# okieraised/rs-face-detection-tflite

Measured on AMD Instinct MI355X. Metric: faces/sec at batch=256 (256x256 back-camera) per GPU, higher is better.
Workload: dtype f32

## Files before the change

### rs-face-detection-tflite_amd/csrc/chain_kernels.hip

```cpp
#include <hip/hip_runtime.h>

#include <algorithm>
#include <cstdint>
#include <type_traits>

#include "kernels.hpp"
#include "launch.hpp"

namespace mi {

typedef float f32x16c __attribute__((ext_vector_type(16)));
typedef float f32x2c __attribute__((ext_vector_type(2)));

namespace {

__device__ __forceinline__ float4 cld4(const float* p) { return *reinterpret_cast<const float4*>(p); }

struct ChainGeom {
    int Cp, Ch, C4, PS, RS, MT;
    int off_wdw, off_bdw, off_bias, off_alpha;
    int split;
    int pre_P, pre_RP, pre_GP, pre_PS, pre_RS;
    int off_t8;
    int lds_bytes;
    unsigned long long* stamps;
};
#ifdef MI_CHAIN_STAMPS
unsigned long long* g_chain_stamps = nullptr;
#define MI_CHAIN_STAMP(k) if (g.stamps && threadIdx.x == 0) { __builtin_amdgcn_sched_barrier(0); g.stamps[(long)blockIdx.x * 24 + (k)] = __builtin_amdgcn_s_memtime(); __builtin_amdgcn_sched_barrier(0); }
#else
#define MI_CHAIN_STAMP(k)
#endif

constexpr int chain_pre_passes(int C, int H, int W, int Cin, int post_Co, int MT, bool split, long tile) {
    const int pre_RS = (2 * W + 1) * (Cin + 4);
    for (int P = 1; P <= 4; P++) {
        const int RP = (H + P - 1) / P, GP = (RP * W + 31) / 32;
        const long stage = (long)(2 * RP + 1) * pre_RS;
        const long rest = 9 * C + C + 8 * 32 + 64 + (post_Co ? (long)(H >> 1) * (W >> 1) * (post_Co + 4) : 0);
        if ((P - 1) * RP < H && P * GP * (split ? MT : 1) <= 8 && ((stage > tile ? stage : tile) + rest) * 4 <= 160 * 1024 - 256) return P;
    }
    return 0;
}

struct GeomRun {
// ... 21 lines not shown
    static constexpr bool all_res = true;
    struct K {
        static constexpr int C = C_, H = H_, W = W_, Cp = C, Ch = C / 2, C4 = C / 4, PS = C + 4, RS = (W + 2) * PS, MT = (C + 31) / 32;
        static constexpr bool split = MT > 1 && ((H * W + 31) / 32) * MT <= 8;
        static constexpr int pre_on = CIN != 0, pre_Cin = CIN, post_on = CO != 0, post_Co = CO;
        static constexpr int tile = (H + 2) * RS;
        static constexpr int pre_PS = CIN + 4, pre_RS = (2 * W + 1) * pre_PS;
        static constexpr int pre_P = CIN ? chain_pre_passes(C, H, W, CIN, CO, MT, split, tile) : 0;
        static constexpr int pre_RP = CIN ? (H + pre_P - 1) / pre_P : 0, pre_GP = (pre_RP * W + 31) / 32;
        static constexpr int stage = CIN ? (2 * pre_RP + 1) * pre_RS : 0;
        static constexpr int off_wdw = stage > tile ? stage : tile, off_bdw = off_wdw + 9 * Cp, off_bias = (off_bdw + Cp + 3) & ~3;
        static constexpr int off_alpha = off_bias + MT * 32;
    };
    static_assert(!CIN || K::pre_P > 0, "no staging plan for `pre`");
    __device__ GeomFixed(const ChainArgs&, const ChainGeom&) {}
#define MI_GEOM_FIELD(f) static constexpr __device__ int f() { return K::f; }
    MI_GEOM_FIELD(C) MI_GEOM_FIELD(H) MI_GEOM_FIELD(W) MI_GEOM_FIELD(pre_on) MI_GEOM_FIELD(pre_Cin) MI_GEOM_FIELD(post_on) MI_GEOM_FIELD(post_Co)
    MI_GEOM_FIELD(Cp) MI_GEOM_FIELD(Ch) MI_GEOM_FIELD(C4) MI_GEOM_FIELD(PS) MI_GEOM_FIELD(RS)
    MI_GEOM_FIELD(off_wdw) MI_GEOM_FIELD(off_bdw) MI_GEOM_FIELD(off_bias) MI_GEOM_FIELD(off_alpha)
    MI_GEOM_FIELD(pre_P) MI_GEOM_FIELD(pre_RP) MI_GEOM_FIELD(pre_GP) MI_GEOM_FIELD(pre_PS) MI_GEOM_FIELD(pre_RS)
#undef MI_GEOM_FIELD
    static bool matches(const ChainArgs& a, const ChainGeom& g) {
        bool ok = a.C == K::C && a.H == K::H && a.W == K::W && g.Cp == K::Cp && g.Ch == K::Ch && g.C4 == K::C4 && g.PS == K::PS && g.RS == K::RS &&
                  g.MT == K::MT && (g.split != 0) == K::split && g.off_wdw == K::off_wdw && g.off_bdw == K::off_bdw && g.off_bias == K::off_bias &&
                  g.off_alpha == K::off_alpha && (a.pre.on != 0) == (CIN != 0) && (a.post.on != 0) == (CO != 0);
        if (ok && CIN) ok = a.pre.Cin == CIN && g.pre_P == K::pre_P && g.pre_RP == K::pre_RP && g.pre_GP == K::pre_GP && g.pre_PS == K::pre_PS && g.pre_RS == K::pre_RS;
        if (ok && CO) ok = a.post.Co == CO;
        for (int k = 0; ok && k < a.nblocks; k++) ok = a.blocks[k].has_res != 0;
        return ok;
    }
};
constexpr int kActRun = -1;

template <int MT, bool SPLIT, class GP = GeomRun, int ACT = kActRun>
__global__ __launch_bounds__(512, 2) void chain_kernel(ChainArgs a, ChainGeom g) {
    extern __shared__ __attribute__((aligned(16))) float lds[];
    const GP geo(a, g);
    float* tile = lds;
    const int tid = threadIdx.x, lane = tid & 63, wave = tid >> 6;
    const int pl = lane & 31, h = lane >> 5;
    const int b = blockIdx.x;
    const float* in = a.in + (long)b * a.in_fs;
    const int rowf4 = geo.W() * geo.C4();
    const int nch = geo.Ch() >> 2;

    struct ConstRegs { float w[3], bdw, bias, alpha; };
    auto fetch_consts = [&](const ChainBlock& cb, int Cs, int Cos, ConstRegs& r) {
#pragma unroll
        for (int k = 0; k < 3; k++) {
            const int i = tid + 512 * k, c = i % geo.Cp();
            r.w[k] = (i < 9 * geo.Cp() && c < Cs) ? cb.w_dw[(i / geo.Cp()) * Cs + c] : 0.f;
        }
        r.bdw = (tid < Cs && cb.b_dw) ? cb.b_dw[tid] : 0.f;
        r.bias = (tid < Cos && cb.bias) ? cb.bias[tid] : 0.f;
        if constexpr (ACT == kActRun) r.alpha = (tid < Cos && cb.act == ACT_PRELU) ? cb.alpha[tid] : (cb.act == ACT_NONE ? 1.f : 0.f);
    };
    auto commit_consts = [&](const ConstRegs& r) {
#pragma unroll
        for (int k = 0; k < 3; k++)
            if (tid + 512 * k < 9 * geo.Cp()) lds[geo.off_wdw() + tid + 512 * k] = r.w[k];
        if (tid < geo.Cp()) lds[geo.off_bdw() + tid] = r.bdw;
        if (tid < MT * 32) {
            lds[geo.off_bias() + tid] = r.bias;
            if constexpr (ACT == kActRun) lds[geo.off_alpha() + tid] = r.alpha;
        }
    };
    unsigned aoff[MT];
// ... 63 lines not shown
        };
        if constexpr (kPeel) step(0, std::true_type{});
        for (int j = kPeel ? 1 : 0; j + 1 < nchk; j++) step(j, std::false_type{});
        mfma_chunk(av, bf, D, std::false_type{});
    };
    constexpr int NJ = MT * 4;
    auto contract1 = [&](const float* w_pw, int nchk, int mt, auto&& dw, f32x16c& D1) {
        const float* wa = w_pw + ((long)mt * nchk * 64 + lane) * 4;
        float4 aw[NJ];
#pragma unroll
        for (int j = 0; j < NJ; j++)
            if (j < nchk) aw[j] = cld4(wa + 256 * j);
        if constexpr (!GP::fixed) {
#pragma unroll
            for (int e = 0; e < 16; e++) D1[e] = 0.f;
        }
        float4 bf;
        dw(0, bf);
#pragma unroll
        for (int j = 0; j < NJ; j++)
            if (j < nchk) {
                float4 bn = bf;
                int jn = j + 1;
                asm volatile("" : "+s"(jn));
                if (j + 1 < nchk) dw(jn, bn);
                if (GP::fixed && j == 0) D1 = __builtin_amdgcn_mfma_f32_32x32x2f32(aw[j].x, bf.x, zero16, 0, 0, 0);
                else D1 = __builtin_amdgcn_mfma_f32_32x32x2f32(aw[j].x, bf.x, D1, 0, 0, 0);
                D1 = __builtin_amdgcn_mfma_f32_32x32x2f32(aw[j].y, bf.y, D1, 0, 0, 0);
                D1 = __builtin_amdgcn_mfma_f32_32x32x2f32(aw[j].z, bf.z, D1, 0, 0, 0);
                D1 = __builtin_amdgcn_mfma_f32_32x32x2f32(aw[j].w, bf.w, D1, 0, 0, 0);
                bf = bn;
                __builtin_amdgcn_sched_barrier(0);
            }
    };
    auto finish1 = [&](f32x16c& D1, int ch, int gq, const float4& skip, float hi) {
        if constexpr (ACT == ACT_RELU) {
            const f32x2c* bb = reinterpret_cast<const f32x2c*>(lds + geo.off_bias() + ch);
            const f32x2c v0 = (f32x2c{D1[4 * gq], D1[4 * gq + 1]} + bb[0]) + f32x2c{skip.x, skip.y};
            const f32x2c v1 = (f32x2c{D1[4 * gq + 2], D1[4 * gq + 3]} + bb[1]) + f32x2c{skip.z, skip.w};
            D1[4 * gq] = fmaxf(v0.x, 0.f);
            D1[4 * gq + 1] = fmaxf(v0.y, 0.f);
            D1[4 * gq + 2] = fmaxf(v1.x, 0.f);
            D1[4 * gq + 3] = fmaxf(v1.y, 0.f);
            return;
        }
        const float4 bb = cld4(lds + geo.off_bias() + ch), al = cld4(lds + geo.off_alpha() + ch);
        const float4 v = make_float4(D1[4 * gq] + bb.x + skip.x, D1[4 * gq + 1] + bb.y + skip.y, D1[4 * gq + 2] + bb.z + skip.z, D1[4 * gq + 3] + bb.w + skip.w);
        D1[4 * gq] = fminf(fmaxf(v.x, 0.f) + al.x * fminf(v.x, 0.f), hi);
        D1[4 * gq + 1] = fminf(fmaxf(v.y, 0.f) + al.y * fminf(v.y, 0.f), hi);
        D1[4 * gq + 2] = fminf(fmaxf(v.z, 0.f) + al.z * fminf(v.z, 0.f), hi);
        D1[4 * gq + 3] = fminf(fmaxf(v.w, 0.f) + al.w * fminf(v.w, 0.f), hi);
    };
    const float4 zero4 = make_float4(0.f, 0.f, 0.f, 0.f);

    const int ngrp = (geo.H() * geo.W() + 31) >> 5;
    const int grp_w = SPLIT ? wave % ngrp : wave, mt_w = SPLIT ? wave / ngrp : 0;
    const int q = grp_w * 32 + pl;
    const bool valid = q < geo.H() * geo.W();
    const int oy = valid ? q / geo.W() : 0, ox = valid ? q - (q / geo.W()) * geo.W() : 0;
    const bool wave_active = SPLIT ? wave < ngrp * MT : wave * 32 < geo.H() * geo.W();
    const int base0 = oy * geo.RS() + ox * geo.PS() + h * geo.Ch();
    float* centre = tile + (oy + 1) * geo.RS() + (ox + 1) * geo.PS();

    MI_CHAIN_STAMP(0)
    ConstRegs cr;
    if (geo.pre_on()) {
// ... 17 lines not shown
            if (p) __syncthreads();
            for (int i = tid; i < nrows * rowf4i; i += 512) {
                const int rr = i / rowf4i, e = i - rr * rowf4i, px = e / C4i, c4 = e - px * C4i, iy = 2 * r0 + rr;
                *reinterpret_cast<float4*>(lds + rr * RSi + px * PSi + 4 * c4) = iy < Hi ? cld4(src + ((long)iy * rowf4i + e) * 4) : zero4;
            }
            for (int i = tid; i < nrows * C4i; i += 512) {
                const int rr = i / C4i, c4 = i - rr * C4i;
                *reinterpret_cast<float4*>(lds + rr * RSi + Wi * PSi + 4 * c4) = zero4;
            }
            __syncthreads();
            MI_CHAIN_STAMP(16 + p)
            const int u = wave - p * UP;
            if (u >= 0 && u < UP) {
                const int ugrp = SPLIT ? u % geo.pre_GP() : u, umt = SPLIT ? u / geo.pre_GP() : 0;
                const int qp = ugrp * 32 + pl;
                const bool vp = qp < (r1 - r0) * geo.W();
                const int oyl = vp ? qp / geo.W() : 0, oxp = vp ? qp - (qp / geo.W()) * geo.W() : 0;
                const float* t0 = lds + (2 * oyl) * RSi + (2 * oxp) * PSi;
                auto dw = [&](int j, float4& bf) {
                    const int c0 = h * Chp + 4 * j;
                    bf = cld4(bdw + c0);
#pragma unroll
                    for (int ky = 0; ky < 3; ky++)
#pragma unroll
                        for (int kx = 0; kx < 3; kx++) {
                            const float4 w = cld4(wdw + (ky * 3 + kx) * geo.Cp() + c0);
                            const float4 d = cld4(t0 + ky * RSi + kx * PSi + c0);
                            bf.x = fmaf(d.x, w.x, bf.x);
                            bf.y = fmaf(d.y, w.y, bf.y);
                            bf.z = fmaf(d.z, w.z, bf.z);
                            bf.w = fmaf(d.w, w.w, bf.w);
                        }
                };
                if constexpr (SPLIT) contract1(cb.w_pw, Chp >> 2, umt, dw, D[0]);
                else contract(cb, Chp >> 2, dw, D);
                const float hi = cb.act == ACT_RELU6 ? 6.f : INFINITY;
#pragma unroll
                for (int m = 0; m < (SPLIT ? 1 : MT); m++)
#pragma unroll
                    for (int gq = 0; gq < 4; gq++) {
                        const int ch = (SPLIT ? umt : m) * 32 + 8 * gq + 4 * h;
                        if (ch >= geo.C()) continue;
                        float4 sk = zero4;
                        if (cb.has_res && ch < Cin) {
                            const float4 s0 = cld4(t0 + ch), s1 = cld4(t0 + PSi + ch), s2 = cld4(t0 + RSi + ch), s3 = cld4(t0 + RSi + PSi + ch);
                            sk = make_float4(fmaxf(fmaxf(s0.x, s1.x), fmaxf(s2.x, s3.x)), fmaxf(fmaxf(s0.y, s1.y), fmaxf(s2.y, s3.y)),
                                             fmaxf(fmaxf(s0.z, s1.z), fmaxf(s2.z, s3.z)), fmaxf(fmaxf(s0.w, s1.w), fmaxf(s2.w, s3.w)));
                        }
                        finish1(D[m], ch, gq, sk, hi);
                    }
                mine = vp;
                my_mt = umt;
                my_centre = tile + (r0 + oyl + 1) * geo.RS() + (oxp + 1) * geo.PS();
            }
        }
        __syncthreads();
        for (int i = tid; i < ((geo.H() + 2) * geo.RS()) >> 2; i += 512) reinterpret_cast<float4*>(tile)[i] = zero4;
        commit_consts(cr);
        __syncthreads();
        if (mine) {
#pragma unroll
            for (int m = 0; m < (SPLIT ? 1 : MT); m++)
#pragma unroll
                for (int gq = 0; gq < 4; gq++) {
                    const int ch = (SPLIT ? my_mt : m) * 32 + 8 * gq + 4 * h;
                    if (ch < geo.C()) *reinterpret_cast<float4*>(my_centre + ch) = make_float4(D[m][4 * gq], D[m][4 * gq + 1], D[m][4 * gq + 2], D[m][4 * gq + 3]);
                }
// ... 35 lines not shown
                        for (int kx = 0; kx < 3; kx++) {
                            const float4 w = cld4(wj + (ky * 3 + kx) * geo.Cp());
                            const float4 d = cld4(tj + ky * geo.RS() + kx * geo.PS());
                            lo = __builtin_elementwise_fma(f32x2c{d.x, d.y}, f32x2c{w.x, w.y}, lo);
                            up = __builtin_elementwise_fma(f32x2c{d.z, d.w}, f32x2c{w.z, w.w}, up);
                        }
                    const float4 bb = cld4(wj + 9 * geo.Cp());
                    lo += f32x2c{bb.x, bb.y};
                    up += f32x2c{bb.z, bb.w};
                    bf = make_float4(lo.x, lo.y, up.x, up.y);
                    return;
                }
                const float* wj = wdw + h * geo.Ch() + 4 * j;
                bf = zero4;
#ifdef MI_ABL_CHAIN_NODW
                bf = cld4(tile + base0 + geo.RS() + geo.PS() + 4 * j);
                return;
#endif
#pragma unroll
                for (int ky = 0; ky < 3; ky++)
#pragma unroll
                    for (int kx = 0; kx < 3; kx++) {
                        const float4 w = cld4(wj + (ky * 3 + kx) * geo.Cp());
                        const float4 d = cld4(tile + base0 + ky * geo.RS() + kx * geo.PS() + 4 * j);
                        bf.x = fmaf(d.x, w.x, bf.x);
                        bf.y = fmaf(d.y, w.y, bf.y);
                        bf.z = fmaf(d.z, w.z, bf.z);
                        bf.w = fmaf(d.w, w.w, bf.w);
                    }
                const float4 bb = cld4(bdw + h * geo.Ch() + 4 * j);
                bf.x += bb.x; bf.y += bb.y; bf.z += bb.z; bf.w += bb.w;
            };
            const float hi = cb.act == ACT_RELU6 ? 6.f : INFINITY;
            if constexpr (SPLIT) contract1(cb.w_pw, nch, mt_w, dw, D[0]);
            else contract(cb, nch, dw, D);
#pragma unroll
            for (int m = 0; m < (SPLIT ? 1 : MT); m++)
#pragma unroll
                for (int gq = 0; gq < 4; gq++) {
                    const int ch = (SPLIT ? mt_w : m) * 32 + 8 * gq + 4 * h;
                    if (ch < geo.C()) finish1(D[m], ch, gq, (GP::all_res || cb.has_res) ? cld4(centre + ch) : zero4, hi);
                }
        }
        __syncthreads();
        if (more || geo.post_on()) commit_consts(cr);
        if (wave_active && valid) {
#pragma unroll
            for (int m = 0; m < (SPLIT ? 1 : MT); m++)
#pragma unroll
                for (int gq = 0; gq < 4; gq++) {
                    const int ch = (SPLIT ? mt_w : m) * 32 + 8 * gq + 4 * h;
                    if (ch < geo.C()) *reinterpret_cast<float4*>(centre + ch) = make_float4(D[m][4 * gq], D[m][4 * gq + 1], D[m][4 * gq + 2], D[m][4 * gq + 3]);
                }
        }
        __syncthreads();
        MI_CHAIN_STAMP(2 + blk)
    }
    if (a.write_out) {
        float* out = a.out + (long)b * a.out_fs;
        for (int i = tid; i < geo.H() * rowf4; i += 512) {
            int r = i / rowf4, e = i - r * rowf4;
            int px = e / geo.C4(), c4 = e - px * geo.C4();
            *reinterpret_cast<float4*>(out + 4 * (long)i) = cld4(tile + (r + 1) * geo.RS() + (px + 1) * geo.PS() + 4 * c4);
        }
    }
    MI_CHAIN_STAMP(10)
    int post_units = 0;
    if (geo.post_on()) {
        const ChainBlock& cb = a.post.blk;
        const int Ho = geo.H() >> 1, Wo = geo.W() >> 1, Co = geo.post_Co(), npo = Ho * Wo;
        const float* wdw = lds + geo.off_wdw();
        const float* bdw = lds + geo.off_bdw();
        const int ngo = (npo + 31) >> 5, MTo = (Co + 31) >> 5;
        post_units = ngo * MTo;
        for (int u = wave; u < post_units; u += 8) {
            const int grp = u % ngo, mt = u / ngo;
            const int qo = grp * 32 + pl;
            const bool vo = qo < npo;
            const int py = vo ? qo / Wo : 0, px = vo ? qo - (qo / Wo) * Wo : 0;
            const float* t0 = tile + (2 * py + 1) * geo.RS() + (2 * px + 1) * geo.PS();
            f32x16c D1;
            auto dw = [&](int j, float4& bf) {
                const int c0 = h * geo.Ch() + 4 * j;
                bf = cld4(bdw + c0);
#pragma unroll
                for (int ky = 0; ky < 3; ky++)
#pragma unroll
                    for (int kx = 0; kx < 3; kx++) {
                        const float4 w = cld4(wdw + (ky * 3 + kx) * geo.Cp() + c0);
                        const float4 d = cld4(t0 + ky * geo.RS() + kx * geo.PS() + c0);
                        bf.x = fmaf(d.x, w.x, bf.x);
                        bf.y = fmaf(d.y, w.y, bf.y);
                        bf.z = fmaf(d.z, w.z, bf.z);
                        bf.w = fmaf(d.w, w.w, bf.w);
                    }
            };
            contract1(cb.w_pw, nch, mt, dw, D1);
            const float hi = cb.act == ACT_RELU6 ? 6.f : INFINITY;
            float* dst = a.post.out + (long)b * a.post.out_fs + (long)qo * Co;
#pragma unroll
            for (int gq = 0; gq < 4; gq++) {
                const int ch = mt * 32 + 8 * gq + 4 * h;
                if (ch >= Co) continue;
                float4 sk = zero4;
                if (cb.has_res && ch < geo.C()) {
                    const float4 s0 = cld4(t0 + ch), s1 = cld4(t0 + geo.PS() + ch), s2 = cld4(t0 + geo.RS() + ch), s3 = cld4(t0 + geo.RS() + geo.PS() + ch);
                    sk = make_float4(fmaxf(fmaxf(s0.x, s1.x), fmaxf(s2.x, s3.x)), fmaxf(fmaxf(s0.y, s1.y), fmaxf(s2.y, s3.y)),
                                     fmaxf(fmaxf(s0.z, s1.z), fmaxf(s2.z, s3.z)), fmaxf(fmaxf(s0.w, s1.w), fmaxf(s2.w, s3.w)));
                }
                finish1(D1, ch, gq, sk, hi);
                if (vo) {
                    const float4 v = make_float4(D1[4 * gq], D1[4 * gq + 1], D1[4 * gq + 2], D1[4 * gq + 3]);
                    *reinterpret_cast<float4*>(dst + ch) = v;
                    if (g.off_t8 >= 0) *reinterpret_cast<float4*>(lds + g.off_t8 + qo * (Co + 4) + ch) = v;
                }
            }
        }
    }
    MI_CHAIN_STAMP(11)
    for (int hd = 0; hd < kChainHeads; hd++) {
        MI_CHAIN_STAMP(12 + hd)
        const ChainHead& H = a.heads[hd];
        if (!H.on) continue;
        if (H.src == 1) { __syncthreads(); post_units = 0; }
        const bool from_post = H.src == 1;
        const int Wh = from_post ? geo.W() >> 1 : geo.W(), np = from_post ? (geo.H() >> 1) * (geo.W() >> 1) : geo.H() * geo.W();
        const int Cs = from_post ? geo.post_Co() : geo.C(), Chs = Cs >> 1, nchs = Chs >> 2;
        const int Cot = H.Co_a + H.Co_b, MTh = (Cot + 31) >> 5, ng = (np + 31) >> 5;
        for (int u = (wave - post_units) & 7; u < ng * MTh; u += 8) {
            const int grp = u % ng, mt = u / ng;
// ... 49 lines not shown
    off = (off + 3) & ~3;
    g.off_bias = off; off += g.MT * 32;
    g.off_alpha = off; off += g.MT * 32;
    g.off_t8 = -1;
    for (int hd = 0; hd < kChainHeads; hd++) {
        const ChainHead& H = a.heads[hd];
        if (!H.on) continue;
        if (H.Co_a < 4 || H.Co_a % 4 || H.Co_b < 0 || H.Co_a + H.Co_b > 128 || !H.out_a || (H.Co_b && !H.out_b) || !H.w_pw) return false;
        if ((reinterpret_cast<uintptr_t>(H.out_a) & 15) || (H.out_a_fs & 3) || (reinterpret_cast<uintptr_t>(H.w_pw) & 15)) return false;
        if (H.src == 1) {
            if (!a.post.on) return false;
            if (g.off_t8 < 0) { g.off_t8 = off; off += (a.H >> 1) * (a.W >> 1) * (a.post.Co + 4); }
        }
    }
    g.lds_bytes = off * 4;
    if (g.lds_bytes > 160 * 1024 - 256) return false;
    auto aligned16 = [](const void* p) { return (reinterpret_cast<uintptr_t>(p) & 15) == 0; };
    if (!aligned16(a.in) || !aligned16(a.out) || (a.in_fs & 3) || (a.out_fs & 3)) return false;
    if (a.pre.on && (a.pre.Cin % 8 || a.pre.Cin < 8 || a.pre.Cin > a.C || !aligned16(a.pre.in) || (a.pre.in_fs & 3))) return false;
    if (a.post.on && ((a.H & 1) || (a.W & 1) || a.post.Co % 4 || a.post.Co < a.C || a.post.Co > g.MT * 32 || !aligned16(a.post.out) || (a.post.out_fs & 3))) return false;
    *out = g;
    return true;
}

using Geom16 = GeomFixed<96, 16, 16, 48, 96>;
using Geom8 = GeomFixed<96, 8, 8, 0, 0>;

bool all_relu(const ChainArgs& a) {
    bool ok = (!a.pre.on || a.pre.blk.act == ACT_RELU) && (!a.post.on || a.post.blk.act == ACT_RELU);
    for (int k = 0; ok && k < a.nblocks; k++) ok = a.blocks[k].act == ACT_RELU;
    return ok;
}

template <int MT, bool SPLIT, class GP = GeomRun, int ACT = kActRun>
int launch_chain_inst(const ChainArgs& a, const ChainGeom& g, hipStream_t s) {
    auto kern = chain_kernel<MT, SPLIT, GP, ACT>;
    if (hipError_t e = allow_full_lds(reinterpret_cast<const void*>(kern)); e != hipSuccess) return (int)e;
    return (int)launch_kernel(kern, dim3((unsigned)a.B), dim3(512), (size_t)g.lds_bytes, s, a, g);
}

}

bool chain_kernel_supports(const ChainArgs& a) {
    ChainGeom g;
    return make_chain_geom(a, &g);
}

int launch_chain(const ChainArgs& a, void* stream, int fixed) {
    ChainGeom g;
    if (!make_chain_geom(a, &g)) return (int)hipErrorInvalidValue;
#ifdef MI_CHAIN_STAMPS
    g.stamps = g_chain_stamps;
#endif
    hipStream_t s = (hipStream_t)stream;
    if (fixed && all_relu(a)) {
        if (Geom16::matches(a, g)) return launch_chain_inst<3, false, Geom16, ACT_RELU>(a, g, s);
        if (Geom8::matches(a, g)) return launch_chain_inst<3, true, Geom8, ACT_RELU>(a, g, s);
    }
    switch (g.MT) {
        case 1: return launch_chain_inst<1, false>(a, g, s);
        case 2: return g.split ? launch_chain_inst<2, true>(a, g, s) : launch_chain_inst<2, false>(a, g, s);
        case 3: return g.split ? launch_chain_inst<3, true>(a, g, s) : launch_chain_inst<3, false>(a, g, s);
        case 4: return g.split ? launch_chain_inst<4, true>(a, g, s) : launch_chain_inst<4, false>(a, g, s);
    }
    return (int)hipErrorInvalidValue;
}

}

#ifdef MI_CHAIN_STAMPS
extern "C" void mi_debug_set_chain_stamps(unsigned long long* p) { mi::g_chain_stamps = p; }
#endif
```

### rs-face-detection-tflite_amd/csrc/engine.cpp

```cpp
#include "engine.hpp"
#include "launch.hpp"

#include <algorithm>
#include <cstdio>
#include <cstdlib>
#include <cstring>
#include <stdexcept>

namespace mi {

void hip_check(hipError_t e, const char* what) {
    if (e != hipSuccess) throw std::runtime_error(std::string(what) + ": " + hipGetErrorString(e));
}

namespace {
template <class T>
void upload(T*& dev, std::vector<T>& host, const char* what_alloc, const char* what_copy) {
    if (dev) hip_check(hipFree(dev), "hipFree");
    dev = nullptr;
    if (host.empty()) return;
    hip_check(hipMalloc(reinterpret_cast<void**>(&dev), host.size() * sizeof(T)), what_alloc);
    hip_check(hipMemcpy(dev, host.data(), host.size() * sizeof(T), hipMemcpyHostToDevice), what_copy);
    std::vector<T>().swap(host);
}
// ... 40 lines not shown

struct Model::Option {
    enum { kReplan = 1,
           kFreeSmall = 2,
           kKeepGraphs = 4,
           kOneOf = 8,
           kKiB = 16 , kWriteOnly = 32, kReadOnly = 64,
           kBandGen = 128,
           kForms = 256 };
    const char* key;
    int Model::*field;
    int lo, hi, flags;
};

const Model::Option* Model::find_option(const std::string& key) {
    using O = Option;
    constexpr int kMax = 0x7fffffff;
    static const Option table[] = {
        {"chunk", &Model::chunk_, 0, kMax, 0},
        {"graph", &Model::use_graph_, 0, 1, 0},
        {"fuse", &Model::fuse_level_, 0, 5, O::kReplan},
        {"res_budget", &Model::res_budget_, 16, 156, O::kReplan | O::kKiB},
        {"pipe", &Model::pipe_max_, 0, 4, O::kReplan},
        {"small_chain", &Model::small_chain_, 0, 64, O::kFreeSmall},
        {"pipe_rows", &Model::pipe_rows_, 1 << 1 | 1 << 2 | 1 << 4, 0, O::kOneOf},
        {"pipe_band", &Model::pipe_band_, 0, 4096, 0},
        {"strip", &Model::strip_, 0, 1, 0},
        {"stem_fuse", &Model::stem_fuse_, 0, 1, 0},
        {"stem_mfma", &Model::stem_mfma_, 0, 2, O::kForms},
        {"stem_run", &Model::stem_run_, 0, 32, 0},
        {"pair_fuse", &Model::pair_fuse_, 0, 1, 0},
        {"mdb_band", &Model::mdb_band_, 0, 4096, 0},
        {"chain_fixed", &Model::chain_fixed_, 0, 1, 0},
        {"mchain", &Model::mchain_, 0, 1, 0},
        {"tail", &Model::tail_, 0, 1, O::kReplan},
        {"tail_pre", &Model::tail_pre_, 0, 2, 0},
        {"tail_g", &Model::tail_g_, 0, 64, 0},
        {"band", &Model::band_, 0, 2, O::kReplan},
        {"band_test_fail", &Model::band_test_fail_, 0, 1, O::kWriteOnly},
        {"band_test_absent", &Model::band_test_absent_, 0, 256, O::kWriteOnly},
        {"band_test_gen", nullptr, 0, kMax, O::kBandGen | O::kWriteOnly},
        {"band_wide", &Model::band_wide_ok_, 0, 1, O::kReplan},
        {"band_fork", &Model::band_fork_, 0, 1, O::kReplan},
        {"band_nw", &Model::band_nw_, 8, 256, O::kReplan},
        {"band_fail_streak", &Model::band_fail_streak_, 0, 0, O::kReadOnly},
        {"band_wraps", &Model::band_wraps_, 0, 0, O::kReadOnly},
        {"fork", &Model::fork_, 0, 1, 0},
        {"heads", &Model::head_streams_opt_, 1, kHeadStreams, O::kReplan},
        {"reuse", &Model::reuse_, 0, 1, O::kReplan},
        {"lanes", &Model::lanes_, 1, 4, 0},
        {"test_poison", &Model::test_poison_, 1 << 1 | 1 << 2, 0, O::kOneOf | O::kKeepGraphs},
    };
    for (const Option& o : table)
        if (key == o.key) return &o;
    return nullptr;
}

void Model::set_option(const std::string& key, int value) {
    const Option* o = find_option(key);
    if (!o || (o->flags & Option::kReadOnly)) throw std::runtime_error("unknown option '" + key + "'");
    int v = (o->lo == 0 && o->hi == 1) ? value != 0 : std::min(o->hi, std::max(o->lo, value));
    if (o->flags & Option::kOneOf) v = (value >= 0 && value < 31 && (o->lo >> value & 1)) ? value : 0;
    if (o->flags & Option::kForms) v = (value >= o->lo && value <= o->hi) ? value : 1;
    if (o->flags & Option::kKiB) v *= 1024;
    if (o->flags & Option::kBandGen) { band_gen_ = static_cast<unsigned>(v); band_gen_force_ = true; }
    else this->*o->field = v;
// ... 178 lines not shown
        st.macs += macs;
        auto dims = [](const std::vector<int>& sh) {
            std::string d;
            for (size_t q = 1; q < sh.size(); q++) d += (q > 1 ? "x" : "") + std::to_string(sh[q]);
            return d;
        };
        if (static_cast<int>(i) == first.launches[k].node) st.detail = dims(si) + "->";
        st.detail = st.detail.substr(0, st.detail.find("->") + 2) + dims(so);
    }
    return stats;
}

LaunchCtx Model::launch_ctx(const float* in, int chunk_start, int frames) const {
    LaunchCtx c;
    c.weights = d_weights_;
    c.arena = d_arena_ + static_cast<size_t>(plan_.arena_floats_per_frame) * chunk_cap_ * arena_lane_;
    c.in = in; c.out = d_out_.data();
    c.small = d_small_; c.small_floats = small_floats_;
    c.progs = d_programs_; c.tail_progs = d_tail_programs_;
    c.band_prog = d_band_prog_; c.band_consts = d_band_consts_; c.band_ws = d_band_ws_; c.band_sync = d_band_sync_; c.band_fail = d_band_fail_;
    c.chunk_cap = chunk_cap_; c.chunk_start = chunk_start; c.F = frames;
    c.u8_frames = u8_.frames; c.u8_lut = u8_.lut; c.u8_frame_bytes = u8_.frame_bytes; c.u8_row_bytes = u8_.row_bytes;
    c.strip = strip_; c.pair_fuse = pair_fuse_; c.stem_fuse = stem_fuse_; c.stem_mfma = stem_mfma_; c.stem_run = stem_run_; c.mchain = mchain_;
    c.small_chain = small_chain_; c.lanes = lanes_;
    c.pipe_rows = pipe_rows_; c.pipe_band = pipe_band_; c.mdb_band = mdb_band_; c.tail_pre = tail_pre_; c.tail_g = tail_g_;
    c.fork = fork_ && lanes_ == 1;
    c.cu_count = device_cu_count();
    c.band = band_use_ && chunk_start == 0;
    c.band_test_absent = band_test_absent_;
    return c;
}

namespace {
int issue(const Launch& l, hipStream_t s, int chain_fixed) {
    auto many = [&](int (*f)(const BlockArgs*, int, void*)) { return f(l.blocks.data(), static_cast<int>(l.blocks.size()), s); };
    switch (l.to) {
        case Launcher::Conv: return launch_conv(std::get<ConvArgs>(l.args), s);
        case Launcher::HeadGemm: return launch_head_gemm(std::get<HeadGemmArgs>(l.args), s);
        case Launcher::Dw: return launch_dw(std::get<DwArgs>(l.args), s);
        case Launcher::Xc: return launch_xc(std::get<XcArgs>(l.args), s);
        case Launcher::Mdblock: return launch_mdblock(std::get<DblockArgs>(l.args), s);
        case Launcher::Dblock: return launch_dblock(std::get<DblockArgs>(l.args), s);
        case Launcher::Mbneck: return launch_mbneck(std::get<BneckArgs>(l.args), s);
        case Launcher::Bneck: return launch_bneck(std::get<BneckArgs>(l.args), s);
        case Launcher::Tail: return launch_tail(std::get<TailLaunch>(l.args), s);
        case Launcher::Resident: return launch_resident(std::get<ResLaunch>(l.args), s);
        case Launcher::Chain: return launch_chain(std::get<ChainArgs>(l.args), s, chain_fixed);
        case Launcher::StripPipe: return many(launch_strip_pipe);
        case Launcher::MstripChain: return many(launch_mstrip_chain);
        case Launcher::SmallChain: {
            int rc = 0;
            for (size_t k = 0; k < l.blocks.size() && rc == 0; k++) rc = l.blocks[k].sh == 1 ? launch_strip(l.blocks[k], s) : launch_block(l.blocks[k], s);
            return rc;
        }
        case Launcher::Ms2: return launch_ms2(std::get<BlockArgs>(l.args), s);
        case Launcher::Mwalk: return launch_mwalk(std::get<BlockArgs>(l.args), s);
        case Launcher::Strip: return launch_strip(std::get<BlockArgs>(l.args), s);
        case Launcher::Mstrip: return launch_mstrip(std::get<BlockArgs>(l.args), s);
        case Launcher::Block: return launch_block(std::get<BlockArgs>(l.args), s);
        case Launcher::Add: return launch_add(std::get<EltArgs>(l.args), s);
        case Launcher::Act: return launch_act(std::get<EltArgs>(l.args), s);
        case Launcher::Maxpool: return launch_maxpool(std::get<EltArgs>(l.args), s);
        case Launcher::Padc: return launch_padc(std::get<EltArgs>(l.args), s);
        case Launcher::Resize2x: return launch_resize2x(std::get<EltArgs>(l.args), s);
        case Launcher::DepthToSpace: return launch_depth_to_space(std::get<EltArgs>(l.args), s);
        case Launcher::Bandnet: return launch_bandnet(std::get<BandLaunch>(l.args), s);
    }
    return 0;
}
}

void Model::enqueue_chunk(const float* in, int chunk_start, int F, hipStream_t trunk, std::vector<hipEvent_t>* marks, Lowered* keep) {
    LaunchCtx ctx = launch_ctx(in, chunk_start, F);
    if (marks) ctx.fork = false;
    Lowered low = lower_chunk(plan_, consts_, band_plan_, sched_, ctx, keep != nullptr);
    auto mark = [&] {
        if (!marks) return;
        hipEvent_t ev;
        hip_check(hipEventCreate(&ev), "hipEventCreate");
        hip_check(hipEventRecord(ev, trunk), "hipEventRecord");
        marks->push_back(ev);
    };
    mark();
    const size_t n_launches = low.launches.size(), start_event = plan_.nodes.size();
    auto event = [&](size_t k) {
        if (head_events_.size() < plan_.nodes.size() + 2 + kHeadStreams) head_events_.resize(plan_.nodes.size() + 2 + kHeadStreams, nullptr);
        if (!head_events_[k]) hip_check(hipEventCreateWithFlags(&head_events_[k], hipEventDisableTiming), "hipEventCreate");
        return head_events_[k];
    };
    unsigned used_heads = 0;
    for (size_t k = 0; k < n_launches; k++) {
        const Launch& l = low.launches[k];
        hipStream_t s = trunk;
        if (l.slot >= 0) {
            while (static_cast<int>(head_streams_.size()) <= l.slot) {
                hipStream_t st;
                hip_check(hipStreamCreateWithFlags(&st, hipStreamNonBlocking), "hipStreamCreate");
                head_streams_.push_back(st);
            }
            s = head_streams_[static_cast<size_t>(l.slot)];
            if (l.wait >= 0) {
                hip_check(wait_event(s, event(static_cast<size_t>(low.launch_of_node[static_cast<size_t>(l.wait)]))), "hipStreamWaitEvent");
            } else {
                hip_check(record_event(event(start_event), trunk), "hipEventRecord");
                hip_check(wait_event(s, event(start_event)), "hipStreamWaitEvent");
            }
            used_heads |= 1u << l.slot;
        }
        int rc = 0;
        for (int rep = 0; rep < (marks ? profile_inner_ : 1) && rc == 0; rep++) rc = issue(l, s, chain_fixed_);
        if (rc != 0) throw std::runtime_error(std::string("kernel launch failed: ") + hipGetErrorString(static_cast<hipError_t>(rc)));
        if (l.record) hip_check(record_event(event(k), s), "hipEventRecord");
        mark();
    }
    for (int k = 0; k < kHeadStreams; k++)
        if (used_heads & (1u << k)) {
            hip_check(record_event(event(start_event + 1 + static_cast<size_t>(k)), head_streams_[static_cast<size_t>(k)]), "hipEventRecord");
            hip_check(wait_event(trunk, event(start_event + 1 + static_cast<size_t>(k))), "hipStreamWaitEvent");
        }
    last_chunk_frames_ = F;
    if (keep) *keep = std::move(low);
}

void Model::enqueue_all(const float* in, int batch, hipStream_t s) {
    if (lanes_ > 1 && batch > chunk_cap_) {
        while (static_cast<int>(side_streams_.size()) < lanes_ - 1) {
            hipStream_t st;
            hip_check(hipStreamCreateWithFlags(&st, hipStreamNonBlocking), "hipStreamCreate");
            side_streams_.push_back(st);
        }
        while (static_cast<int>(lane_events_.size()) < lanes_) {
            hipEvent_t ev;
            hip_check(hipEventCreateWithFlags(&ev, hipEventDisableTiming), "hipEventCreate");
            lane_events_.push_back(ev);
        }
        hip_check(record_event(lane_events_[0], s), "hipEventRecord");
        int lane = 0;
        for (int start = 0; start < batch; start += chunk_cap_, lane = (lane + 1) % lanes_) {
            hipStream_t ls = lane == 0 ? s : side_streams_[lane - 1];
            if (lane > 0 && start < chunk_cap_ * lanes_) hip_check(wait_event(ls, lane_events_[0]), "hipStreamWaitEvent");
            arena_lane_ = lane;
            enqueue_chunk(in, start, std::min(chunk_cap_, batch - start), ls);
        }
// ... 187 lines not shown
```

### rs-face-detection-tflite_amd/csrc/engine.hpp

```cpp
#pragma once

#include <hip/hip_runtime.h>

#include <map>
#include <memory>
#include <string>
#include <vector>

#include "bandplan.hpp"
#include "consts.hpp"
#include "launches.hpp"
#include "plan.hpp"

namespace mi {

void hip_check(hipError_t e, const char* what);

class Model {
   public:
    Model(const uint8_t* bytes, size_t n, int device);
    ~Model();
    Model(const Model&) = delete;
    Model& operator=(const Model&) = delete;

// ... 17 lines not shown
    void run_device_u8(const uint8_t* frames, long frame_bytes, int row_bytes, const float* lut, int batch, hipStream_t stream);

    struct LaunchStat {
        std::string kernel, detail;
        double ms = 0, bytes = 0, macs = 0;
    };
    std::vector<LaunchStat> profile(const float* in, int batch, int reps, hipStream_t stream);
    void set_option(const std::string& key, int value);
    size_t debug_tensor(int tensor, int frame, float* dst, size_t cap);
    std::string describe() const { return plan_.describe(); }

   private:
    void rebuild();
    struct Option;
    static const Option* find_option(const std::string& key);
    void build_bandnet();
    void free_bandnet();
    bool band_usable(int batch) const;
    void band_before_launch(hipStream_t s);
    void poison_scratch(hipStream_t s);
    void ensure_capacity(int batch);
    LaunchCtx launch_ctx(const float* in, int chunk_start, int frames) const;
    void enqueue_chunk(const float* in, int chunk_start, int frames, hipStream_t s, std::vector<hipEvent_t>* marks = nullptr, Lowered* keep = nullptr);
    void enqueue_all(const float* in, int batch, hipStream_t s);
    void invalidate_graphs();

    int device_ = 0;
    std::vector<uint8_t> blob_;
    Plan plan_;
    int fuse_level_ = 5, pipe_max_ = 4, tail_ = 1, reuse_ = 1;
    int res_budget_ = 156 * 1024;
    int chunk_ = 0, lanes_ = 1, use_graph_ = 1;
    int fork_ = 1, head_streams_opt_ = 1;
    int strip_ = 1, stem_fuse_ = 1, stem_mfma_ = 1, stem_run_ = 0, pair_fuse_ = 1, mchain_ = 1, chain_fixed_ = 1;
    int pipe_rows_ = 0, pipe_band_ = 0, mdb_band_ = 0;
    int tail_pre_ = 0, tail_g_ = 0;
    int arena_lane_ = 0;
    std::vector<hipStream_t> side_streams_;
    std::vector<hipEvent_t> lane_events_;
    SideSchedule sched_;
    std::vector<hipStream_t> head_streams_;
    std::vector<hipEvent_t> head_events_;
    bool dirty_ = true;

    float* d_weights_ = nullptr;
    PlanConsts consts_;
    int profile_inner_ = 1;

    ResStage* d_programs_ = nullptr;
    TailStage* d_tail_programs_ = nullptr;
    float* d_arena_ = nullptr;
    size_t arena_floats_ = 0;
    int chunk_cap_ = 0;
    int batch_cap_ = 0;
    std::vector<float*> d_out_;
    float* d_in_stage_ = nullptr;
    size_t in_stage_floats_ = 0;
    int last_chunk_frames_ = 0;

    int band_ = 1;
    int band_nw_ = 128;
    BandPlan band_plan_;
    bool band_use_ = false;
    bool band_ran_ = false;
    int band_test_fail_ = 0;
    int band_test_absent_ = 0;
    int test_poison_ = 0;
// ... 44 lines not shown
```

### rs-face-detection-tflite_amd/csrc/kernels.hpp

```cpp
#pragma once

#include <cstddef>
#include <cstdint>

namespace mi {

enum ActKind : int { ACT_NONE = 0, ACT_RELU = 1, ACT_RELU6 = 2, ACT_PRELU = 3 };
enum ResMode : int { RES_NONE = 0, RES_DIRECT = 1, RES_MAXPOOL = 2, RES_UP2X = 3 };

struct Epilogue {
    const float* bias = nullptr;
    const float* alpha = nullptr;
    const float* res = nullptr;
    long res_fs = 0;
    int res_mode = RES_NONE;
    int res_C = 0;
    int res_W = 0, res_H = 0;
    int act = ACT_NONE;
    int res_after = 0;
};

struct ConvArgs {
    const float* in = nullptr;
    const uint8_t* in_u8 = nullptr;
// ... 238 lines not shown
bool strip_kernel_supports(const BlockArgs& a);
bool strip_shape_ok(int C, int Co);
int strip_consts_floats(int C);
void strip_pack_consts(int C, const float* w_dw, const float* b_dw, const float* w_pw, const float* bias, const float* alpha, int act, float* dst);
const char* strip_kernel_label(const BlockArgs& a, char* buf, size_t cap);
int launch_mwalk(const BlockArgs& a, void* stream);
bool mwalk_kernel_supports(const BlockArgs& a);
bool mwalk_shape_ok(int W, int C, int Co);
int mwalk_consts_floats(int W, int C, int Co);
void mwalk_pack_consts(int W, int C, int Co, const float* w_dw, const float* b_dw, const float* w_pw, const float* bias, const float* alpha, int act, float* dst);
const char* mwalk_kernel_label(const BlockArgs& a, char* buf, size_t cap);
int launch_ms2(const BlockArgs& a, void* stream);
bool ms2_kernel_supports(const BlockArgs& a);
bool ms2_shape_ok(int W, int C, int Co, bool skip);
int ms2_consts_floats(int W, int C, int Co, bool skip);
void ms2_pack_consts(int W, int C, int Co, bool skip, const float* w_dw, const float* b_dw, const float* w_pw, const float* bias, const float* alpha, int act, float* dst);
const char* ms2_kernel_label(const BlockArgs& a, char* buf, size_t cap);
int launch_mstrip(const BlockArgs& a, void* stream);
bool mstrip_kernel_supports(const BlockArgs& a);
bool mstrip_shape_ok(int C, int Co);
int mstrip_consts_floats(int C);
void mstrip_pack_consts(int C, const float* w_dw, const float* b_dw, const float* w_pw, const float* bias, const float* alpha, int act, float* dst);
const char* mstrip_kernel_label(const BlockArgs& a, char* buf, size_t cap);
bool mstrip_chain_supports(const BlockArgs* blocks, int n);
int launch_mstrip_chain(const BlockArgs* blocks, int n, void* stream);
bool strip_pipe_supports(const BlockArgs* blocks, int n);
bool strip_pipe_shape_ok(int C, int W);
bool strip_tail_shape_ok(int C, int Co, int H, int W);
int strip_consts_s2_floats(int C, int Co);
void strip_pack_consts_s2(int C, int Co, const float* w_dw, const float* b_dw, const float* w_pw, const float* bias, const float* alpha, int act, float* dst);
int launch_strip_pipe(const BlockArgs* blocks, int n, void* stream);
const char* strip_pipe_label(const BlockArgs* blocks, int n, char* buf, size_t cap);
int strip_pipe_rows_per_step(int H, int hint = 0);
int launch_chain(const ChainArgs& a, void* stream, int fixed = 1);

struct BneckBlock {
    const float* w1 = nullptr;
    const float* w2 = nullptr;
    const float* consts = nullptr;
    float hi1 = 0.f, hi2 = 0.f;
    const float* mconsts = nullptr;
    int act1 = ACT_RELU, act2 = ACT_RELU;
};
constexpr int kMaxBneck = 6;
struct BneckArgs {
    const float* in = nullptr;
    float* out = nullptr;
    long in_fs = 0, out_fs = 0;
    int B = 0, H = 0, W = 0, C = 0, Cm = 0, nblocks = 0;
    int bands = 1;
    BneckBlock blocks[kMaxBneck];
};
struct XcStage {
    const float* cblob = nullptr;
    int has_dw = 1;
    const float* w_pw = nullptr;
    int C = 0, Co = 0;
    int act = ACT_RELU;
    int skip = 0;
    const float* res = nullptr;
    long res_fs = 0;
    int res_C = 0, res_W = 0;
};
constexpr int kMaxXc = 8;
struct XcArgs {
    const float* in = nullptr;
    float* out = nullptr;
// ... 135 lines not shown
```

Before: 219,300.

## Software-pipeline depthwise LDS reads against MFMA in fixed-geometry chain kernels

Adds a hand-scheduled contraction path for the fixed-geometry chain kernels. Depthwise taps and weights for the next channel chunk are issued as inline-asm ds_read_b128 loads with immediate offsets, and the current chunk's MFMAs run before waiting on them. The goal is to hide LDS latency behind the pointwise MFMA work and drop per-tap address arithmetic. In exchange it holds more vector registers live, uses explicit waitcnt and sched barriers, and is enabled by default through a new chain_sched option.

```diff
diff --git a/rs-face-detection-tflite_amd/csrc/chain_kernels.hip b/rs-face-detection-tflite_amd/csrc/chain_kernels.hip
--- a/rs-face-detection-tflite_amd/csrc/chain_kernels.hip
+++ b/rs-face-detection-tflite_amd/csrc/chain_kernels.hip
@@ -11,6 +11,7 @@
 
 typedef float f32x16c __attribute__((ext_vector_type(16)));
 typedef float f32x2c __attribute__((ext_vector_type(2)));
+typedef float f32x4c __attribute__((ext_vector_type(4)));
 
 namespace {
 
@@ -98,7 +99,40 @@
 };
 constexpr int kActRun = -1;
 
-template <int MT, bool SPLIT, class GP = GeomRun, int ACT = kActRun>
+struct DwTaps { f32x4c w[9], d[9], b; };
+template <int WS_, int RSB_, int PSB_, bool BIAS_FIRST_>
+struct DwForm { static constexpr int WS = WS_, RSB = RSB_, PSB = PSB_; static constexpr bool bias_first = BIAS_FIRST_; };
+template <int OFF>
+__device__ __forceinline__ void lds_request(unsigned addr, f32x4c& v) { asm volatile("ds_read_b128 %0, %1 offset:%2" : "=v"(v) : "v"(addr), "n"(OFF)); }
+template <class F, int... K>
+__device__ __forceinline__ void dw_request(unsigned wa, unsigned ta, DwTaps& t, std::integer_sequence<int, K...>) {
+    static_assert(9 * F::WS + 16 * 16 < 65536 && 2 * F::RSB + 2 * F::PSB + 16 * 16 < 65536, "ds_read offsets are 16 bits");
+    ((lds_request<K * F::WS>(wa, t.w[K]), lds_request<(K / 3) * F::RSB + (K % 3) * F::PSB>(ta, t.d[K])), ...);
+    lds_request<9 * F::WS>(wa, t.b);
+}
+template <class F>
+__device__ __forceinline__ void dw_request(unsigned wa, unsigned ta, DwTaps& t) { dw_request<F>(wa, ta, t, std::make_integer_sequence<int, 9>{}); }
+__device__ __forceinline__ void dw_landed(DwTaps& t) {
+    asm volatile("s_waitcnt lgkmcnt(0)" ::: "memory");
+#pragma unroll
+    for (int k = 0; k < 9; k++) asm volatile("" : "+v"(t.w[k]), "+v"(t.d[k]));
+    asm volatile("" : "+v"(t.b));
+}
+template <bool BIAS_FIRST>
+__device__ __forceinline__ void dw_fma(const DwTaps& t, float4& bf) {
+    f32x2c lo = {0.f, 0.f}, up = {0.f, 0.f};
+    if constexpr (BIAS_FIRST) { lo = f32x2c{t.b.x, t.b.y}; up = f32x2c{t.b.z, t.b.w}; }
+#pragma unroll
+    for (int k = 0; k < 9; k++) {
+        lo = __builtin_elementwise_fma(f32x2c{t.d[k].x, t.d[k].y}, f32x2c{t.w[k].x, t.w[k].y}, lo);
+        up = __builtin_elementwise_fma(f32x2c{t.d[k].z, t.d[k].w}, f32x2c{t.w[k].z, t.w[k].w}, up);
+    }
+    if constexpr (!BIAS_FIRST) { lo += f32x2c{t.b.x, t.b.y}; up += f32x2c{t.b.z, t.b.w}; }
+    asm volatile("" : "+v"(lo), "+v"(up));
+    bf = make_float4(lo.x, lo.y, up.x, up.y);
+}
+
+template <int MT, bool SPLIT, class GP = GeomRun, int ACT = kActRun, int SCHED = 0>
 __global__ __launch_bounds__(512, 2) void chain_kernel(ChainArgs a, ChainGeom g) {
     extern __shared__ __attribute__((aligned(16))) float lds[];
     const GP geo(a, g);
@@ -228,6 +262,74 @@
                 bf = bn;
                 __builtin_amdgcn_sched_barrier(0);
             }
+    };
+    [[maybe_unused]] auto lds_addr = [](const float* p) { return (unsigned)(uintptr_t)(__attribute__((address_space(3))) float*)const_cast<float*>(p); };
+    [[maybe_unused]] auto contract_ph = [&](auto form, auto nchk_c, const ChainBlock& cb, unsigned wa, unsigned ta, auto& D) {
+        using F = decltype(form);
+        constexpr int NCH = decltype(nchk_c)::value;
+        static_assert(NCH >= 4 && NCH % 2 == 0, "chunks are taken in pairs: the weight fragments alternate between two register sets");
+        DwTaps t;
+        float4 bf, av[2][MT];
+        a_frag(cb, NCH, 0, av[0]);
+        dw_request<F>(wa, ta, t);
+        dw_landed(t);
+        dw_fma<F::bias_first>(t, bf);
+        auto step = [&](int j, const float4 (&ac)[MT], float4 (&an)[MT], auto first, auto last) {
+            if constexpr (!decltype(last)::value) {
+                a_frag(cb, NCH, j + 1, an);
+                dw_request<F>(wa + 16u * (unsigned)(j + 1), ta + 16u * (unsigned)(j + 1), t);
+            }
+            __builtin_amdgcn_sched_barrier(0);
+            mfma_chunk(ac, bf, D, first);
+            __builtin_amdgcn_sched_barrier(0);
+            if constexpr (!decltype(last)::value) {
+#pragma unroll
+                for (int m = 0; m < MT; m++) asm volatile("" : "+v"(D[m]));
+                dw_landed(t);
+                dw_fma<F::bias_first>(t, bf);
+                __builtin_amdgcn_sched_barrier(0);
+            }
+        };
+        step(0, av[0], av[1], std::true_type{}, std::false_type{});
+        for (int j = 1; j + 2 < NCH; j += 2) {
+            step(j, av[1], av[0], std::false_type{}, std::false_type{});
+            step(j + 1, av[0], av[1], std::false_type{}, std::false_type{});
+        }
+        step(NCH - 1, av[1], av[1], std::false_type{}, std::true_type{});
+    };
+    [[maybe_unused]] auto contract1_ph = [&](auto form, auto nchk_c, const float* w_pw, int mt, unsigned wa, unsigned ta, f32x16c& D1) {
+        using F = decltype(form);
+        constexpr int NCH = decltype(nchk_c)::value;
+        const float* wag = w_pw + ((long)mt * NCH * 64 + lane) * 4;
+        float4 aw[NCH];
+#pragma unroll
+        for (int j = 0; j < NCH; j++) aw[j] = cld4(wag + 256 * j);
+        DwTaps t;
+        float4 bf;
+        dw_request<F>(wa, ta, t);
+        dw_landed(t);
+        dw_fma<F::bias_first>(t, bf);
+#pragma unroll
+        for (int j = 0; j < NCH; j++) {
+            if (j + 1 < NCH) {
+                unsigned jn = 16u * (unsigned)(j + 1);
+                asm volatile("" : "+s"(jn));
+                dw_request<F>(wa + jn, ta + jn, t);
+            }
+            __builtin_amdgcn_sched_barrier(0);
+            if (j == 0) D1 = __builtin_amdgcn_mfma_f32_32x32x2f32(aw[j].x, bf.x, zero16, 0, 0, 0);
+            else D1 = __builtin_amdgcn_mfma_f32_32x32x2f32(aw[j].x, bf.x, D1, 0, 0, 0);
+            D1 = __builtin_amdgcn_mfma_f32_32x32x2f32(aw[j].y, bf.y, D1, 0, 0, 0);
+            D1 = __builtin_amdgcn_mfma_f32_32x32x2f32(aw[j].z, bf.z, D1, 0, 0, 0);
+            D1 = __builtin_amdgcn_mfma_f32_32x32x2f32(aw[j].w, bf.w, D1, 0, 0, 0);
+            __builtin_amdgcn_sched_barrier(0);
+            if (j + 1 < NCH) {
+                asm volatile("" : "+v"(D1));
+                dw_landed(t);
+                dw_fma<F::bias_first>(t, bf);
+                __builtin_amdgcn_sched_barrier(0);
+            }
+        }
     };
     auto finish1 = [&](f32x16c& D1, int ch, int gq, const float4& skip, float hi) {
         if constexpr (ACT == ACT_RELU) {
@@ -311,7 +413,11 @@
                             bf.w = fmaf(d.w, w.w, bf.w);
                         }
                 };
-                if constexpr (SPLIT) contract1(cb.w_pw, Chp >> 2, umt, dw, D[0]);
+                if constexpr (SCHED == 1 && !SPLIT) {
+                    using K = typename GP::K;
+                    contract_ph(DwForm<K::Cp * 4, K::pre_RS * 4, K::pre_PS * 4, true>{}, std::integral_constant<int, K::pre_Cin / 8>{}, cb,
+                                lds_addr(wdw + h * Chp), lds_addr(t0 + h * Chp), D);
+                } else if constexpr (SPLIT) contract1(cb.w_pw, Chp >> 2, umt, dw, D[0]);
                 else contract(cb, Chp >> 2, dw, D);
                 const float hi = cb.act == ACT_RELU6 ? 6.f : INFINITY;
 #pragma unroll
@@ -413,7 +519,13 @@
                 bf.x += bb.x; bf.y += bb.y; bf.z += bb.z; bf.w += bb.w;
             };
             const float hi = cb.act == ACT_RELU6 ? 6.f : INFINITY;
-            if constexpr (SPLIT) contract1(cb.w_pw, nch, mt_w, dw, D[0]);
+            if constexpr (SCHED == 1) {
+                using K = typename GP::K;
+                using F = DwForm<K::Cp * 4, K::RS * 4, K::PS * 4, false>;
+                using N = std::integral_constant<int, K::Ch / 4>;
+                if constexpr (SPLIT) contract1_ph(F{}, N{}, cb.w_pw, mt_w, lds_addr(lds + wlane), lds_addr(tile + base0), D[0]);
+                else contract_ph(F{}, N{}, cb, lds_addr(lds + wlane), lds_addr(tile + base0), D);
+            } else if constexpr (SPLIT) contract1(cb.w_pw, nch, mt_w, dw, D[0]);
             else contract(cb, nch, dw, D);
 #pragma unroll
             for (int m = 0; m < (SPLIT ? 1 : MT); m++)
@@ -476,7 +588,11 @@
                         bf.w = fmaf(d.w, w.w, bf.w);
                     }
             };
-            contract1(cb.w_pw, nch, mt, dw, D1);
+            if constexpr (SCHED == 1) {
+                using K = typename GP::K;
+                contract1_ph(DwForm<K::Cp * 4, K::RS * 4, K::PS * 4, true>{}, std::integral_constant<int, K::Ch / 4>{}, cb.w_pw, mt,
+                             lds_addr(wdw + h * geo.Ch()), lds_addr(t0 + h * geo.Ch()), D1);
+            } else contract1(cb.w_pw, nch, mt, dw, D1);
             const float hi = cb.act == ACT_RELU6 ? 6.f : INFINITY;
             float* dst = a.post.out + (long)b * a.post.out_fs + (long)qo * Co;
 #pragma unroll
@@ -592,9 +708,9 @@
     return ok;
 }
 
-template <int MT, bool SPLIT, class GP = GeomRun, int ACT = kActRun>
+template <int MT, bool SPLIT, class GP = GeomRun, int ACT = kActRun, int SCHED = 0>
 int launch_chain_inst(const ChainArgs& a, const ChainGeom& g, hipStream_t s) {
-    auto kern = chain_kernel<MT, SPLIT, GP, ACT>;
+    auto kern = chain_kernel<MT, SPLIT, GP, ACT, SCHED>;
     if (hipError_t e = allow_full_lds(reinterpret_cast<const void*>(kern)); e != hipSuccess) return (int)e;
     return (int)launch_kernel(kern, dim3((unsigned)a.B), dim3(512), (size_t)g.lds_bytes, s, a, g);
 }
@@ -606,7 +722,7 @@
     return make_chain_geom(a, &g);
 }
 
-int launch_chain(const ChainArgs& a, void* stream, int fixed) {
+int launch_chain(const ChainArgs& a, void* stream, int fixed, int sched) {
     ChainGeom g;
     if (!make_chain_geom(a, &g)) return (int)hipErrorInvalidValue;
 #ifdef MI_CHAIN_STAMPS
@@ -614,8 +730,8 @@
 #endif
     hipStream_t s = (hipStream_t)stream;
     if (fixed && all_relu(a)) {
-        if (Geom16::matches(a, g)) return launch_chain_inst<3, false, Geom16, ACT_RELU>(a, g, s);
-        if (Geom8::matches(a, g)) return launch_chain_inst<3, true, Geom8, ACT_RELU>(a, g, s);
+        if (Geom16::matches(a, g)) return sched ? launch_chain_inst<3, false, Geom16, ACT_RELU, 1>(a, g, s) : launch_chain_inst<3, false, Geom16, ACT_RELU, 0>(a, g, s);
+        if (Geom8::matches(a, g)) return sched ? launch_chain_inst<3, true, Geom8, ACT_RELU, 1>(a, g, s) : launch_chain_inst<3, true, Geom8, ACT_RELU, 0>(a, g, s);
     }
     switch (g.MT) {
         case 1: return launch_chain_inst<1, false>(a, g, s);
diff --git a/rs-face-detection-tflite_amd/csrc/engine.cpp b/rs-face-detection-tflite_amd/csrc/engine.cpp
--- a/rs-face-detection-tflite_amd/csrc/engine.cpp
+++ b/rs-face-detection-tflite_amd/csrc/engine.cpp
@@ -96,6 +96,7 @@
         {"pair_fuse", &Model::pair_fuse_, 0, 1, 0},
         {"mdb_band", &Model::mdb_band_, 0, 4096, 0},
         {"chain_fixed", &Model::chain_fixed_, 0, 1, 0},
+        {"chain_sched", &Model::chain_sched_, 0, 1, 0},
         {"mchain", &Model::mchain_, 0, 1, 0},
         {"tail", &Model::tail_, 0, 1, O::kReplan},
         {"tail_pre", &Model::tail_pre_, 0, 2, 0},
@@ -340,7 +341,7 @@
 }
 
 namespace {
-int issue(const Launch& l, hipStream_t s, int chain_fixed) {
+int issue(const Launch& l, hipStream_t s, int chain_fixed, int chain_sched) {
     auto many = [&](int (*f)(const BlockArgs*, int, void*)) { return f(l.blocks.data(), static_cast<int>(l.blocks.size()), s); };
     switch (l.to) {
         case Launcher::Conv: return launch_conv(std::get<ConvArgs>(l.args), s);
@@ -353,7 +354,7 @@
         case Launcher::Bneck: return launch_bneck(std::get<BneckArgs>(l.args), s);
         case Launcher::Tail: return launch_tail(std::get<TailLaunch>(l.args), s);
         case Launcher::Resident: return launch_resident(std::get<ResLaunch>(l.args), s);
-        case Launcher::Chain: return launch_chain(std::get<ChainArgs>(l.args), s, chain_fixed);
+        case Launcher::Chain: return launch_chain(std::get<ChainArgs>(l.args), s, chain_fixed, chain_sched);
         case Launcher::StripPipe: return many(launch_strip_pipe);
         case Launcher::MstripChain: return many(launch_mstrip_chain);
         case Launcher::SmallChain: {
@@ -416,7 +417,7 @@
             used_heads |= 1u << l.slot;
         }
         int rc = 0;
-        for (int rep = 0; rep < (marks ? profile_inner_ : 1) && rc == 0; rep++) rc = issue(l, s, chain_fixed_);
+        for (int rep = 0; rep < (marks ? profile_inner_ : 1) && rc == 0; rep++) rc = issue(l, s, chain_fixed_, chain_sched_);
         if (rc != 0) throw std::runtime_error(std::string("kernel launch failed: ") + hipGetErrorString(static_cast<hipError_t>(rc)));
         if (l.record) hip_check(record_event(event(k), s), "hipEventRecord");
         mark();
diff --git a/rs-face-detection-tflite_amd/csrc/engine.hpp b/rs-face-detection-tflite_amd/csrc/engine.hpp
--- a/rs-face-detection-tflite_amd/csrc/engine.hpp
+++ b/rs-face-detection-tflite_amd/csrc/engine.hpp
@@ -73,7 +73,7 @@
     int res_budget_ = 156 * 1024;
     int chunk_ = 0, lanes_ = 1, use_graph_ = 1;
     int fork_ = 1, head_streams_opt_ = 1;
-    int strip_ = 1, stem_fuse_ = 1, stem_mfma_ = 1, stem_run_ = 0, pair_fuse_ = 1, mchain_ = 1, chain_fixed_ = 1;
+    int strip_ = 1, stem_fuse_ = 1, stem_mfma_ = 1, stem_run_ = 0, pair_fuse_ = 1, mchain_ = 1, chain_fixed_ = 1, chain_sched_ = 1;
     int pipe_rows_ = 0, pipe_band_ = 0, mdb_band_ = 0;
     int tail_pre_ = 0, tail_g_ = 0;
     int arena_lane_ = 0;
diff --git a/rs-face-detection-tflite_amd/csrc/kernels.hpp b/rs-face-detection-tflite_amd/csrc/kernels.hpp
--- a/rs-face-detection-tflite_amd/csrc/kernels.hpp
+++ b/rs-face-detection-tflite_amd/csrc/kernels.hpp
@@ -294,7 +294,7 @@
 int launch_strip_pipe(const BlockArgs* blocks, int n, void* stream);
 const char* strip_pipe_label(const BlockArgs* blocks, int n, char* buf, size_t cap);
 int strip_pipe_rows_per_step(int H, int hint = 0);
-int launch_chain(const ChainArgs& a, void* stream, int fixed = 1);
+int launch_chain(const ChainArgs& a, void* stream, int fixed = 1, int sched = 1);
 
 struct BneckBlock {
     const float* w1 = nullptr;
```

Result: faster. 222,500, median of 6 (+1.4%).
